# SkylerGao/MC_NeRF

Hardware: AMD Instinct MI355X
Metric: train rays/sec (coarse+fine, 64+128 samples) (higher is better)
Workload: dtype f16x3h; 1 GPU; Ball_Lego-shaped 110-view 800x800, coarse 4x128 @64 + fine 8x256 @128-grid, GLOBAL_OPTIM stage, fwd+bwd+allreduce+RAdam; precision=f16x3h, parallelism=dp1

## Files before the change

### mc_nerf_amd/csrc/mcnerf_x3.h

```cpp
#pragma once
#include "mcnerf_16.h"

#define MCNX3_SW 256.0f
#define MCNX3_SX 8.0f
#define MCNX3_SLABF 8
#define MCNX3_PF 2

#define MCNX3_WIDE_MIN 128
static inline constexpr int mcnx3_waves(int width) { return width >= MCNX3_WIDE_MIN ? 4 : 8; }

static inline int mcnx3_pad(int frags) { return (frags + MCNX3_SLABF - 1) / MCNX3_SLABF * MCNX3_SLABF; }
static inline Mcn16Stream mcnx3_repad(Mcn16Stream st) {
    int total = 0;
    for (int s = 0; s < st.nseg; ++s) {
        st.seg[s].first_frag = total;
        total += mcnx3_pad(st.seg[s].tiles * (st.seg[s].a.ksteps + st.seg[s].b.ksteps));
    }
    st.total_frags = total;
    return st;
}
static inline Mcn16Stream mcnx3_fwd_stream(const McnLayout& L) { return mcnx3_repad(mcn16_fwd_stream(L)); }
static inline Mcn16Stream mcnx3_bwd_stream(const McnLayout& L) { return mcnx3_repad(mcn16_bwd_stream(L)); }

static inline size_t mcnx3_slot_bytes(long long capacity, int width) { return 2 * mcn16_slot_bytes(capacity, width); }
static inline size_t mcnx3_enc_bytes(long long capacity) { return 2 * mcn16_enc_bytes(capacity); }
static inline size_t mcnx3_sh_bytes(long long capacity) { return (size_t)mcn16_cap_tiles(capacity) * 4096; }
static inline size_t mcnx3_dsh_bytes(long long capacity) { return 2 * mcn16_dsh_bytes(capacity); }

hipError_t mcnx3_launch_fwd(const Mcn16FwdArgs& a, hipStream_t st);
hipError_t mcnx3_launch_bwd(const Mcn16BwdArgs& a, hipStream_t st);
hipError_t mcnx3_launch_dw(const Mcn16DwArgs& a, hipStream_t st);
hipError_t mcnx3_launch_pack(const McnLayout& L, const float* params, void* packed_fwd, void* packed_bwd, unsigned* range_flags, hipStream_t st);

#ifdef __HIPCC__
typedef float f32x2_t __attribute__((ext_vector_type(2)));

__device__ __forceinline__ void mcnx3_split2(float a, float b, unsigned& hi, unsigned& lo) {
    const f16x2_t h = __builtin_convertvector((f32x2_t){a, b}, f16x2_t);
    const f32x2_t back = __builtin_convertvector(h, f32x2_t);
    const f16x2_t l = __builtin_convertvector((f32x2_t){a - back[0], b - back[1]}, f16x2_t);
    hi = __builtin_bit_cast(unsigned, h);
    lo = __builtin_bit_cast(unsigned, l);
}
__device__ __forceinline__ float mcnx3_val(unsigned hi, unsigned lo, int e) {
    const f16x2_t h = __builtin_bit_cast(f16x2_t, hi), l = __builtin_bit_cast(f16x2_t, lo);
    return (float)h[e] + (float)l[e];
}
template <int HI>
__device__ __forceinline__ float mcnx3_residual(float v, unsigned hw) {
    float r;
    if (HI) asm("v_fma_mix_f32 %0, %1, -1.0, %2 op_sel:[1,0,0] op_sel_hi:[1,0,0]" : "=v"(r) : "v"(hw), "v"(v));
    else asm("v_fma_mix_f32 %0, %1, -1.0, %2 op_sel_hi:[1,0,0]" : "=v"(r) : "v"(hw), "v"(v));
    return r;
}
__device__ __forceinline__ float mcnx3_relu(float x) {
    const int i = __builtin_bit_cast(int, x);
    return __builtin_bit_cast(float, i > 0 ? i : 0);
}
__device__ __forceinline__ f32x16 mcnx3_mfma(const u32x4_t& a, const u32x4_t& b, const f32x16& c) {
    return __builtin_amdgcn_mfma_f32_32x32x16_f16(__builtin_bit_cast(f16x8_t, a), __builtin_bit_cast(f16x8_t, b), c, 0, 0, 0);
}
__device__ __forceinline__ void mcnx3_mfma3(f32x16& acc, const u32x4_t& ah, const u32x4_t& al, const u32x4_t& bh, const u32x4_t& bl) {
    acc = mcnx3_mfma(al, bh, acc);
    acc = mcnx3_mfma(ah, bl, acc);
    acc = mcnx3_mfma(ah, bh, acc);
}

__device__ __forceinline__ void mcnx3_dma16(const char* ubase, unsigned voff, unsigned lds_dst) {
    unsigned keep;
    asm volatile("s_mov_b32 %0, m0\n\ts_mov_b32 m0, %3\n\ts_nop 0\n\tglobal_load_lds_dwordx4 %1, %2\n\ts_mov_b32 m0, %0"
                 : "=&s"(keep) : "v"(voff), "s"(ubase), "s"(lds_dst) : "memory");
}
template <int PPW>
__device__ __forceinline__ void mcnx3_ring_issue(Mcn16Ring& r) {
    const char* s = r.ubase + (size_t)r.src_slab * (MCN16_SLAB * 1024);
    const unsigned d = r.lds_base + r.issue_slot * (MCN16_SLAB * 1024) + r.lds_piece;
#pragma unroll
    for (int i = 0; i < PPW; ++i) mcnx3_dma16(s + i * 1024, r.voff, d + i * 1024);
    r.src_slab = (r.src_slab + 1 == r.n_slabs) ? 0 : r.src_slab + 1;
    r.issue_slot = (r.issue_slot + 1) & (MCN16_RING - 1);
}
template <int PPW>
__device__ __forceinline__ void mcnx3_ring_sync(Mcn16Ring& r) {
    asm volatile("s_waitcnt vmcnt(%0)\n\ts_barrier" ::"n"(PPW * (MCN16_AHEAD - 1)) : "memory");
    r.next_off = r.sync_slot * (MCN16_SLAB * 1024);
    r.sync_slot = (r.sync_slot + 1) & (MCN16_RING - 1);
    mcnx3_ring_issue<PPW>(r);
}
template <int PPW>
__device__ __forceinline__ void mcnx3_ring_start(Mcn16Ring& r, char* ring_lds, const void* packed, int n_slabs, int wave, int lane) {
    r.ubase = reinterpret_cast<const char*>(packed) + (PPW * wave) * 1024;
    r.voff = lane * 16;
    r.src = nullptr;
    r.lds_piece = (PPW * wave) * 1024;
    r.lds_base = (unsigned)reinterpret_cast<size_t>((mcn16_lds_ptr_t)ring_lds);
    r.src_slab = 0; r.n_slabs = n_slabs; r.issue_slot = 0; r.sync_slot = 0; r.next_off = 0;
#pragma unroll
    for (int i = 0; i < MCN16_AHEAD; ++i) mcnx3_ring_issue<PPW>(r);
    mcnx3_ring_sync<PPW>(r);
}
template <int F>
__host__ __device__ constexpr int mcnx3_sync_at(int q) {
    return (MCNX3_SLABF * q + MCNX3_SLABF - MCNX3_PF) < (F - 1) ? (MCNX3_SLABF * q + MCNX3_SLABF - MCNX3_PF) : (F - 1);
}
template <int F, int PPW>
__device__ __forceinline__ void mcnx3_before_mfma(Mcn16Ring& r, Mcn16Cursor& c, int f) {
    if ((f & (MCNX3_SLABF - 1)) == 0) c.cur = r.next_off;
    if (f == mcnx3_sync_at<F>(f / MCNX3_SLABF)) mcnx3_ring_sync<PPW>(r);
}
#define MCNX3_DMA_STEP 2
template <int PPW>
__device__ __forceinline__ void mcnx3_ring_piece(Mcn16Ring& r, int i) {
    switch (i) {
        case 0: asm volatile("global_load_lds_dwordx4 %0, %1" ::"v"(r.voff), "s"(r.piece_base) : "memory"); break;
        case 1: asm volatile("global_load_lds_dwordx4 %0, %1 offset:1024" ::"v"(r.voff), "s"(r.piece_base) : "memory"); break;
        case 2: asm volatile("global_load_lds_dwordx4 %0, %1 offset:2048" ::"v"(r.voff), "s"(r.piece_base) : "memory"); break;
        default: asm volatile("global_load_lds_dwordx4 %0, %1 offset:3072" ::"v"(r.voff), "s"(r.piece_base) : "memory"); break;
    }
// ... 53 lines not shown
```

### mc_nerf_amd/csrc/mlp_x3_bwd.hip

```cpp
#include "mcnerf_x3.h"
#include "mcnerf_launch.h"

#define MCNX3_BWD_PREF_MINW 256
#include <cstdlib>

template <int W>
struct BwdX3Smem {
    static constexpr int WAVES = mcnx3_waves(W);
    static constexpr int oW2 = MCN16_RING * MCN16_SLAB * 1024;
    static constexpr int oBarf = oW2 + W * 4;
    static constexpr int MW = W >= 64 ? W / 64 : 1;
    static constexpr int oMask = oBarf + 16 * 4;
    static constexpr int oIdx = oMask + WAVES * 3 * MW * 256;
    static constexpr int oIn = oIdx + WAVES * 256;
    static constexpr int total = oIn + (W >= 256 ? WAVES * 16 * 256 : 0);
};

template <int W, int KSTEPS, int NTILES, int MODE, int PPW, bool HI>
__device__ __forceinline__ void mcnx3_bwd_seg(Mcn16Ring& ring, char* smem, int lane,
                                              const u32x4_t (&inh)[W / 16], const u32x4_t (&inl)[W / 16],
                                              u32x4_t (&outh)[W / 16], u32x4_t (&outl)[W / 16],
                                              const unsigned (&mk)[W >= 64 ? W / 64 : 1], f32x16 (&acc2)[2], char* save_lane) {
    constexpr int KS = W / 16, F = NTILES * KSTEPS, G = 3 * KSTEPS;
    constexpr bool EPI = MODE != 3;
    constexpr int NIT = EPI ? (MODE == 0 ? 16 : 20) : 0;
    constexpr int START = (G >= NIT + 8) ? 3 : 0;
    constexpr int IPG = EPI ? (NIT + (G - START) - 1) / (G - START) : 1;
    constexpr int LASTA = EPI ? START + 14 / IPG : 0;
    constexpr int SBASE = START + 16, SSTR = (G - SBASE) / 4 > 0 ? (G - SBASE) / 4 : 1;
    constexpr bool STAG = (MODE == 1 || MODE == 2) && IPG == 1 && (G - SBASE) / 4 >= 2;
    constexpr int NITG = STAG ? 16 : NIT;
    constexpr int INIT_G = (G - 8) > LASTA ? (G - 8) : LASTA;
    constexpr int INIT_N = (INIT_G + 3 <= G - 1) ? 4 : 1;
    Mcn16Cursor cur;
    u32x4_t afh[MCNX3_PF], afl[MCNX3_PF];
    f32x16 acc[2];
    float v0 = 0.f, v1 = 0.f;
    unsigned wkeep = 0u;
    auto acc_init = [&](f32x16& a, int t, int q) {
        if (MODE == 2) {
            const f16x8_t h8 = __builtin_bit_cast(f16x8_t, outh[2 * t + (q >> 1)]), l8 = __builtin_bit_cast(f16x8_t, outl[2 * t + (q >> 1)]);
#pragma unroll
            for (int e = 0; e < 4; ++e) a[4 * q + e] = ((float)h8[4 * (q & 1) + e] + (float)l8[4 * (q & 1) + e]) * MCNX3_SW;
        } else {
#pragma unroll
            for (int e = 0; e < 4; ++e) a[4 * q + e] = 0.f;
        }
    };
    auto item = [&](const f32x16& a, int t, int i) {
        if (i < 16) {
            const int p = i >> 1;
            const unsigned bits = MODE != 0 ? ((mk[t >> 1] >> (8 * (t & 1) + 7 - p)) & 0x00010001u) : 0u;
            if ((i & 1) == 0) {
                v0 = a[2 * p] * (1.0f / MCNX3_SW);
                v1 = a[2 * p + 1] * (1.0f / MCNX3_SW);
                const unsigned w = Mcn16T<false>::pack(v0, v1);
                wkeep = w;
                outh[2 * t + (p >> 2)][p & 3] = MODE != 0 ? mcn16_pkmul(w, bits) : w;
            } else {
                const unsigned w = Mcn16T<false>::pack(mcnx3_residual<0>(v0, wkeep), mcnx3_residual<1>(v1, wkeep));
                outl[2 * t + (p >> 2)][p & 3] = MODE != 0 ? mcn16_pkmul(w, bits) : w;
            }
        } else {
            const int k = i - 16, s = 2 * t + (k & 1);
            if (k < 2) mcn16_ws_store(outh[s], reinterpret_cast<u32x4_t*>(save_lane + s * 1024));
            else if (!HI) mcn16_ws_store(outl[s], reinterpret_cast<u32x4_t*>(save_lane + (KS + s) * 1024));
        }
    };
    cur.cur = ring.next_off;
#pragma unroll
    for (int i = 0; i < MCNX3_PF; ++i)
        if (i < F) {
            afh[i] = *reinterpret_cast<const u32x4_t*>(smem + ring.next_off + i * 2048 + lane * 16);
            afl[i] = *reinterpret_cast<const u32x4_t*>(smem + ring.next_off + i * 2048 + 1024 + lane * 16);
        }
    if (EPI) {
#pragma unroll
        for (int q = 0; q < 4; ++q) acc_init(acc[0], 0, q);
    }
#pragma unroll
    for (int t = 0; t < NTILES; ++t) {
#pragma unroll
        for (int s = 0; s < KSTEPS; ++s) {
            const int f = t * KSTEPS + s;
            mcnx3_before_mfma_spread<F, PPW>(ring, cur, f);
            const u32x4_t a_h = afh[f % MCNX3_PF], a_l = afl[f % MCNX3_PF];
            if (f + MCNX3_PF < F) {
                const unsigned o = mcnx3_frag_off(ring, cur, f, f + MCNX3_PF) + lane * 16;
                afh[f % MCNX3_PF] = *reinterpret_cast<const u32x4_t*>(smem + o);
                afl[f % MCNX3_PF] = *reinterpret_cast<const u32x4_t*>(smem + o + 1024);
            }
#pragma unroll
            for (int g = 0; g < 3; ++g) {
                const int gap = 3 * s + g;
                if (EPI && t > 0 && gap >= START) {
#pragma unroll
                    for (int i = (gap - START) * IPG; i < (gap - START + 1) * IPG; ++i)
                        if (i < NITG) item(acc[(t - 1) & 1], t - 1, i);
                    if (STAG && gap >= SBASE && (gap - SBASE) / SSTR < 4 && (gap - SBASE) % SSTR == 0)
                        item(acc[(t - 1) & 1], t - 1, 16 + (gap - SBASE) / SSTR);
                }
                if (EPI && t + 1 < NTILES && gap >= INIT_G && gap < INIT_G + INIT_N) {
#pragma unroll
                    for (int q = 0; q < 4; ++q)
                        if (INIT_N == 1 || q == gap - INIT_G) acc_init(acc[(t + 1) & 1], t + 1, q);
                }
                mcnx3_gap_dma<F, PPW>(ring, 3 * f + g);
                __builtin_amdgcn_sched_barrier(0);
                if (EPI) acc[t & 1] = mcnx3_mfma(g == 0 ? a_l : a_h, g == 1 ? inl[s] : inh[s], acc[t & 1]);
                else acc2[t & 1] = mcnx3_mfma(g == 0 ? a_l : a_h, g == 1 ? inl[s] : inh[s], acc2[t & 1]);
                __builtin_amdgcn_sched_barrier(0);
            }
        }
    }
    mcnx3_layer_end<F, PPW>(ring);
    if (EPI) {
#pragma unroll
        for (int i = 0; i < NIT; ++i) item(acc[(NTILES - 1) & 1], NTILES - 1, i);
    }
}

template <int W, bool HI>
__global__ __launch_bounds__(64 * mcnx3_waves(W), mcnx3_waves(W) / 4) void mlp_x3_bwd_kernel(Mcn16BwdArgs a) {
    using SM = BwdX3Smem<W>;
    constexpr int PL = HI ? 1 : 2;
    constexpr int WAVES = mcnx3_waves(W), ROWS = 32 * WAVES, PPW = 16 / WAVES;
    constexpr int NT = W / 32, KS = W / 16, MW = W >= 64 ? W / 64 : 1;
    extern __shared__ __attribute__((aligned(16))) char smem[];
    const int tid = threadIdx.x, lane = tid & 63, wave = __builtin_amdgcn_readfirstlane(tid >> 6);
    const int m = lane & 31, h = lane >> 5;
    const int D = a.lay.depth, skip = a.lay.skip;
    const long long total = a.count ? (long long)min(*a.count, a.max_rows) : (long long)a.n_rays * a.S;
    if ((long long)blockIdx.x * ROWS >= total) return;

    float* sw2 = reinterpret_cast<float*>(smem + SM::oW2);
    for (int i = tid; i < W; i += 64 * WAVES) sw2[i] = a.params[a.lay.pWs2 + i];
    float* sbarf = reinterpret_cast<float*>(smem + SM::oBarf);
    if (tid < MCN_NFREQ) sbarf[tid] = a.barf_w[tid];
    const float gmax = __uint_as_float(*a.gmax_bits);
    const float sg = mcn16_grad_scale(gmax);
    const float inv_sg = 1.0f / sg;
    __syncthreads();

    struct In { int ray; float zg, jit; f32x4 o, go; float dx, dy, dz, ox, oy, oz; };
    auto gather = [&](int ray, int j) -> In {
        In r;
        r.ray = ray;
        r.zg = a.zgrid[ray * a.z_stride + j];
        r.jit = a.jitter ? a.jitter[ray] : 0.f;
        const size_t addr = (size_t)ray * a.S + j;
        r.o = *reinterpret_cast<const f32x4*>(a.out + addr * 4);
        r.go = *reinterpret_cast<const f32x4*>(a.d_out + addr * 4);
        r.dx = a.rays_d[ray * 3]; r.dy = a.rays_d[ray * 3 + 1]; r.dz = a.rays_d[ray * 3 + 2];
        r.ox = a.rays_o[ray * 3]; r.oy = a.rays_o[ray * 3 + 1]; r.oz = a.rays_o[ray * 3 + 2];
        return r;
    };
    auto row_of = [&](long long pass_) -> long long {
        const long long g_ = (pass_ * WAVES + wave) * 32 + m;
        return g_ < total ? g_ : total - 1;
    };
    constexpr bool PREFB = W >= MCNX3_BWD_PREF_MINW;
    constexpr int SLABS_FULL = (W / 32) * (W / 16) / MCNX3_SLABF;
    constexpr int SLABS_ENC = (2 * (W / 16) + MCNX3_SLABF - 1) / MCNX3_SLABF;
    constexpr int N_IDX = PPW * (2 * SLABS_FULL - 1) < 63 ? PPW * (2 * SLABS_FULL - 1) : 63;
    constexpr int N_TOP = PPW * (SLABS_FULL + SLABS_ENC - 1) < 63 ? PPW * (SLABS_FULL + SLABS_ENC - 1) : 63;
    const unsigned in_lds = (unsigned)reinterpret_cast<size_t>((mcn16_lds_ptr_t)smem) + SM::oIn + wave * (16 * 256);
    const float* in_rd = reinterpret_cast<const float*>(smem + SM::oIn + wave * (16 * 256)) + lane;
    auto gather_dma = [&](int ray, int j) {
        mcn16_dma4(a.zgrid + ray * a.z_stride + j, in_lds);
        if (a.jitter) mcn16_dma4(a.jitter + ray, in_lds + 256);
        const size_t addr = ((size_t)ray * a.S + j) * 4;
#pragma unroll
        for (int c = 0; c < 4; ++c) {
            mcn16_dma4(a.out + addr + c, in_lds + (2 + c) * 256);
            mcn16_dma4(a.d_out + addr + c, in_lds + (6 + c) * 256);
        }
#pragma unroll
        for (int c = 0; c < 3; ++c) {
            mcn16_dma4(a.rays_d + ray * 3 + c, in_lds + (10 + c) * 256);
            mcn16_dma4(a.rays_o + ray * 3 + c, in_lds + (13 + c) * 256);
// ... 95 lines not shown
                unsigned wh, wl;
                mcnx3_split2(v[0], v[1], wh, wl);
                dshh[s][d] = wh; dshl[s][d] = wl;
            }
        {
            char* e = reinterpret_cast<char*>(a.dsh_ws) + (size_t)tile * (PL * 2) * 1024 + lane * 16;
            mcn16_ws_store(dshh[0], reinterpret_cast<u32x4_t*>(e));
            mcn16_ws_store(dshh[1], reinterpret_cast<u32x4_t*>(e + 1024));
            if (!HI) {
                mcn16_ws_store(dshl[0], reinterpret_cast<u32x4_t*>(e + 2048));
                mcn16_ws_store(dshl[1], reinterpret_cast<u32x4_t*>(e + 3072));
            }
        }

        if (MASK_DMA) mask_read(mask_lane, mk_s, 0, D);
        else {
#pragma unroll
            for (int i = 0; i < MW; ++i) { mk_s[i] = mk0_s[i]; mk_c[i] = mk0_c[i]; mk_t[i] = mk0_t[i]; }
        }
        const long long pass_n = pass + gridDim.x;
        if (a.idx) {
            const long long gn = (pass_n * WAVES + wave) * 32 + (lane >> 1);
            mcn16_dma4(reinterpret_cast<const int*>(a.idx) + 2 * (gn < total ? gn : total - 1) + (lane & 1), idx_lds);
        }
        const bool want_rays = a.d_rays_o || a.d_rays_d;
        f32x4 shs[4];
#pragma unroll
        for (int q = 0; q < 4; ++q) shs[q] = f32x4{0.f, 0.f, 0.f, 0.f};
        if (PREFB && want_rays) {
#pragma unroll
            for (int q = 0; q < 4; ++q)
                shs[q] = *reinterpret_cast<const f32x4*>(reinterpret_cast<const char*>(a.sh_ws) + (size_t)tile * 4096 + q * 1024 + lane * 16);
        }
        u32x4_t xah[KS], xal[KS], xbh[KS], xbl[KS];
        f32x16 denc[2];
#pragma unroll
        for (int t = 0; t < 2; ++t)
#pragma unroll
            for (int e = 0; e < 16; ++e) denc[t][e] = 0.f;
#pragma unroll
        for (int s = 0; s < KS; ++s) {
            const f32x4 wa = *reinterpret_cast<const f32x4*>(w2_h + 16 * s), wb = *reinterpret_cast<const f32x4*>(w2_h + 16 * s + 8);
            const int t = s >> 1;
#pragma unroll
            for (int d = 0; d < 4; ++d) {
                const float va = (d < 2 ? wa[2 * d] : wb[2 * d - 4]) * dsg, vb = (d < 2 ? wa[2 * d + 1] : wb[2 * d - 3]) * dsg;
                const int i = 4 * (s & 1) + d;
                const unsigned bits = (mk_s[t >> 1] >> (8 * (t & 1) + 7 - i)) & 0x00010001u;
                unsigned wh, wl;
                mcnx3_split2(va, vb, wh, wl);
                xah[s][d] = mcn16_pkmul(wh, bits);
                xal[s][d] = mcn16_pkmul(wl, bits);
            }
            mcn16_ws_store(xah[s], reinterpret_cast<u32x4_t*>(dy_lane + (size_t)D * a.slot_bytes + s * 1024));
            if (!HI) mcn16_ws_store(xal[s], reinterpret_cast<u32x4_t*>(dy_lane + (size_t)D * a.slot_bytes + (KS + s) * 1024));
        }
        if (D >= 2) mask_issue(mask_lane, D - 2, buf_of(D - 2));
        unsigned mpend[MW];
        if (!MASK_DMA && D >= 2) mask_read(mask_lane, mpend, 0, D - 2);
        mcnx3_bwd_seg<W, KS, NT, 0, PPW, HI>(ring, smem, lane, xah, xal, xbh, xbl, mk_s, denc, nullptr);
        if (MASK_DMA) mask_read(mask_lane, mk_c, 1, D + 1);
        {
            u32x4_t dih[KS], dil[KS];
            dih[0] = dshh[0]; dih[1] = dshh[1]; dil[0] = dshl[0]; dil[1] = dshl[1];
            mcnx3_bwd_seg<W, 2, NT, 1, PPW, HI>(ring, smem, lane, dih, dil, xah, xal, mk_c, denc, dy_lane + (size_t)(D + 1) * a.slot_bytes);
        }
        if (D >= 3) mask_issue(mask_lane, D - 3, buf_of(D - 3));
        if (MASK_DMA) mask_read(mask_lane, mk_t, 2, D - 1);
        mcnx3_bwd_seg<W, KS, NT, 2, PPW, HI>(ring, smem, lane, xah, xal, xbh, xbl, mk_t, denc, dy_lane + (size_t)(D - 1) * a.slot_bytes);
        auto trunk_masks = [&](int l) {
            if (MASK_DMA) {
                if (l >= 3) mask_issue(mask_lane, l - 3, buf_of(l - 3));
                mask_read(mask_lane, mk_t, buf_of(l - 1), l - 1);
            } else {
#pragma unroll
                for (int i = 0; i < MW; ++i) mk_t[i] = mpend[i];
                if (l >= 2) mask_read(mask_lane, mpend, 0, l - 2);
            }
            if (l == 1 && pass_n * ROWS < total) {
                const unsigned* mln = mask_lane_of(pass_n);
                mask_issue(mln, D, 0); mask_issue(mln, D + 1, 1); mask_issue(mln, D - 1, 2);
                if (!MASK_DMA) { mask_read(mln, mk0_s, 0, D); mask_read(mln, mk0_c, 1, D + 1); mask_read(mln, mk0_t, 2, D - 1); }
            }
        };
        auto next_rows = [&]() {
            asm volatile("s_waitcnt vmcnt(%0)" ::"n"(N_IDX) : "memory");
            int rn, jn;
            if (a.idx) {
                const int2 rj = *reinterpret_cast<const int2*>(smem + SM::oIdx + wave * 256 + m * 8);
                rn = rj.x; jn = rj.y;
            } else {
                const long long gn = row_of(pass_n);
                rn = (int)(gn / a.S); jn = (int)(gn - (long long)rn * a.S);
            }
            gather_dma(rn, jn);
            ray_n = rn;
        };
        for (int l = D - 1; l >= 1; l -= 2) {
            if (PREFB && l == 1) next_rows();
            trunk_masks(l);
            if (l == skip) mcnx3_bwd_seg<W, KS, 2, 3, PPW, HI>(ring, smem, lane, xbh, xbl, xah, xal, mk_t, denc, nullptr);
            mcnx3_bwd_seg<W, KS, NT, 1, PPW, HI>(ring, smem, lane, xbh, xbl, xah, xal, mk_t, denc, dy_lane + (size_t)(l - 1) * a.slot_bytes);
            if (l - 1 >= 1) {
                if (PREFB && l - 1 == 1) next_rows();
                trunk_masks(l - 1);
                if (l - 1 == skip) mcnx3_bwd_seg<W, KS, 2, 3, PPW, HI>(ring, smem, lane, xah, xal, xbh, xbl, mk_t, denc, nullptr);
                mcnx3_bwd_seg<W, KS, NT, 1, PPW, HI>(ring, smem, lane, xah, xal, xbh, xbl, mk_t, denc, dy_lane + (size_t)(l - 2) * a.slot_bytes);
            } else {
#pragma unroll
                for (int s = 0; s < KS; ++s) { xbh[s] = xah[s]; xbl[s] = xal[s]; }
            }
        }
        In nxt = cur;
        if (PREFB && D < 2) {
            next_rows();
        }
        if (!PREFB) {
            int rn, jn;
            if (a.idx) {
                const int2 rj = *reinterpret_cast<const int2*>(smem + SM::oIdx + wave * 256 + m * 8);
                rn = rj.x; jn = rj.y;
            } else {
                const long long gn = row_of(pass_n);
                rn = (int)(gn / a.S); jn = (int)(gn - (long long)rn * a.S);
            }
            nxt = gather(rn, jn);
        }
        if (!PREFB && want_rays) {
#pragma unroll
            for (int q = 0; q < 4; ++q)
                shs[q] = *reinterpret_cast<const f32x4*>(reinterpret_cast<const char*>(a.sh_ws) + (size_t)tile * 4096 + q * 1024 + lane * 16);
        }
        mcnx3_bwd_seg<W, KS, 2, 3, PPW, HI>(ring, smem, lane, xbh, xbl, xah, xal, mk_t, denc, nullptr);
        auto settle = [&]() {
            if (PREFB && D >= 2) return;
            asm volatile("s_waitcnt vmcnt(0)" ::: "memory");
            asm volatile("" : "+v"(nxt.ray), "+v"(nxt.zg), "+v"(nxt.jit), "+v"(nxt.o), "+v"(nxt.go));
            asm volatile("" : "+v"(nxt.dx), "+v"(nxt.dy), "+v"(nxt.dz), "+v"(nxt.ox), "+v"(nxt.oy), "+v"(nxt.oz));
            if (!MASK_DMA) {
#pragma unroll
                for (int i = 0; i < MW; ++i) asm volatile("" : "+v"(mk0_s[i]), "+v"(mk0_c[i]), "+v"(mk0_t[i]));
            }
        };

        if (want_rays) {
            auto dch = [&](int ch) -> float {
                const int hh = (ch >> 2) & 1;
                const float v = denc[ch >> 5][4 * ((ch >> 3) & 3) + (ch & 3)];
                return (h == hh) ? v : 0.f;
            };
            float dpos[3];
#pragma unroll
            for (int ax = 0; ax < 3; ++ax) {
                float acc = dch(ax);
                float S[MCN_NFREQ], C[MCN_NFREQ];
                mcn_sincos_octaves<MCN_NFREQ>(p[ax], S, C);
#pragma unroll
                for (int f = 0; f < MCN_NFREQ; ++f) {
                    const float k = (float)(1 << f) * sbarf[f];
                    acc = fmaf(k * C[f], dch(3 + 20 * ax + f), acc);
                    acc = fmaf(-k * S[f], dch(3 + 20 * ax + 10 + f), acc);
                }
                dpos[ax] = acc * (1.0f / MCNX3_SW);
            }
            float ddir[3] = {0.f, 0.f, 0.f};
            {
                const float C1 = 0.4886025119029199f, C20 = 1.0925484305920792f, C22 = 0.31539156525252005f, C24 = 0.5462742152960396f;
                const float gx[9] = {0.f, 0.f, 0.f, -C1, C20 * y, 0.f, -2.f * C22 * x, -C20 * z, 2.f * C24 * x};
                const float gy[9] = {0.f, -C1, 0.f, 0.f, C20 * x, -C20 * z, -2.f * C22 * y, 0.f, -2.f * C24 * y};
                const float gz[9] = {0.f, 0.f, C1, 0.f, 0.f, -C20 * y, 4.f * C22 * z, -C20 * x, 0.f};
#pragma unroll
                for (int r = 0; r < 16; ++r) {
                    const float v = shs[r >> 2][r & 3];
                    const int n0 = 8 * (r >> 2) + (r & 3), n1 = n0 + 4;
                    const float kx = h ? (n1 < MCN_NSH ? dpre[n1 / 9] * gx[n1 % 9] : 0.f) : (n0 < MCN_NSH ? dpre[n0 / 9] * gx[n0 % 9] : 0.f);
                    const float ky = h ? (n1 < MCN_NSH ? dpre[n1 / 9] * gy[n1 % 9] : 0.f) : (n0 < MCN_NSH ? dpre[n0 / 9] * gy[n0 % 9] : 0.f);
                    const float kz = h ? (n1 < MCN_NSH ? dpre[n1 / 9] * gz[n1 % 9] : 0.f) : (n0 < MCN_NSH ? dpre[n0 / 9] * gz[n0 % 9] : 0.f);
                    ddir[0] = fmaf(kx, v, ddir[0]); ddir[1] = fmaf(ky, v, ddir[1]); ddir[2] = fmaf(kz, v, ddir[2]);
                }
            }
            float red[6];
#pragma unroll
            for (int c = 0; c < 3; ++c) {
                const float dp = dpos[c] + __shfl_xor(dpos[c], 32);
                const float dd = ddir[c] + __shfl_xor(ddir[c], 32);
                red[c] = dp * inv_sg;
// ... 40 lines not shown
```

### mc_nerf_amd/csrc/mlp_x3_fwd.hip

```cpp
#include "mcnerf_x3.h"
#include "mcnerf_launch.h"

template <int W>
struct FwdX3Smem {
    static constexpr int oBias = MCN16_RING * MCN16_SLAB * 1024;
    static constexpr int oW2 = oBias + (MCN_MAXD + 2) * W * 4;
    static constexpr int oBc2 = oW2 + W * 4;
    static constexpr int oIdx = oBc2 + 32 * 4;
    static constexpr int oIn = oIdx + mcnx3_waves(W) * 256;
    static constexpr int total = oIn + mcnx3_waves(W) * 8 * 256;
};

template <int W, int SV, int KENC, int KHID, int EPI, int PPW>
__device__ __forceinline__ void mcnx3_layer(Mcn16Ring& ring, char* smem, int lane,
                                            const u32x4_t (&ench)[MCN16_ENCKS], const u32x4_t (&encl)[MCN16_ENCKS],
                                            const u32x4_t (&inh)[W / 16], const u32x4_t (&inl)[W / 16],
                                            u32x4_t (&outh)[W / 16], u32x4_t (&outl)[W / 16], const float* bias_h,
                                            const float* w2_h, float& dot, char* save_lane, unsigned* mask_lane) {
    constexpr bool SAVE = SV != 0, HI = SV == 2;
    constexpr int NT = W / 32, KS = W / 16, KTOT = KENC + KHID, F = NT * KTOT, MW = W >= 64 ? W / 64 : 1;
    constexpr int G = 3 * KTOT;
    constexpr bool HAS2 = SAVE || EPI == 1;
    constexpr int IPW = HAS2 ? 3 : 2;
    constexpr int NST = SAVE ? (HI ? 2 : 4) : 0;
    constexpr int NIT = 8 * IPW + NST;
    constexpr int NWI = 8 * IPW;
    constexpr int ROOM = G - 3 - 2 * NST;
    constexpr int IPGA = ROOM > 0 ? (NWI + ROOM - 1) / ROOM : 99;
    constexpr bool STAG = SAVE && IPGA <= 2;
    constexpr int START = STAG ? 3 : (G >= NIT + 4 ? 3 : 0);
    constexpr int IPG = STAG ? IPGA : (NIT + (G - START) - 1) / (G - START);
    constexpr int NITG = STAG ? NWI : NIT;
    constexpr int LASTG = START + (NITG + IPG - 1) / IPG - 1;
    constexpr int SBASE = LASTG + 1, SSTR = STAG ? (G - SBASE) / NST : 1;
    constexpr int BIAS_G = (G - 6) > LASTG ? (G - 6) : LASTG;
    Mcn16Cursor cur;
    unsigned mw[MW];
#pragma unroll
    for (int i = 0; i < MW; ++i) mw[i] = 0u;
    u32x4_t afh[MCNX3_PF], afl[MCNX3_PF];
    f32x16 acc[2];
    unsigned mb = 0u;
    float v0 = 0.f, v1 = 0.f;
    unsigned wkeep = 0u;
    auto bias_init = [&](f32x16& a, int t) {
#pragma unroll
        for (int q = 0; q < 4; ++q) {
            const f32x4 b = *reinterpret_cast<const f32x4*>(bias_h + 32 * t + 8 * q);
#pragma unroll
            for (int e = 0; e < 4; ++e) a[4 * q + e] = b[e];
        }
    };
    auto item = [&](const f32x16& a, int t, int i) {
        if (i < 8 * IPW) {
            const int p = i / IPW, ph = i % IPW;
            if (ph == 0) {
                v0 = mcnx3_relu(a[2 * p] * (1.0f / MCNX3_SW));
                v1 = mcnx3_relu(a[2 * p + 1] * (1.0f / MCNX3_SW));
                const unsigned w = Mcn16T<false>::pack(v0, v1);
                wkeep = w;
                outh[2 * t + (p >> 2)][p & 3] = w;
            } else if (ph == IPW - 1) {
                outl[2 * t + (p >> 2)][p & 3] = Mcn16T<false>::pack(mcnx3_residual<0>(v0, wkeep), mcnx3_residual<1>(v1, wkeep));
            } else {
                if (SAVE) {
                    mb = (p == 0) ? mcn16_nz(wkeep) : ((mb << 1) | mcn16_nz(wkeep));
                    if (p == 7) mw[t >> 1] |= mb << (8 * (t & 1));
                }
                if (EPI == 1) {
                    const f32x2_t ww = *reinterpret_cast<const f32x2_t*>(w2_h + 32 * t + 8 * (p >> 1) + 2 * (p & 1));
                    dot = fmaf(v0, ww[0], dot);
                    dot = fmaf(v1, ww[1], dot);
                }
            }
        } else if (SAVE) {
            const int k = i - 8 * IPW;
            const int s = 2 * t + (k & 1);
            if (k < 2) mcn16_ws_store(outh[s], reinterpret_cast<u32x4_t*>(save_lane + s * 1024));
            else mcn16_ws_store(outl[s], reinterpret_cast<u32x4_t*>(save_lane + (KS + s) * 1024));
        }
    };
    cur.cur = ring.next_off;
#pragma unroll
    for (int i = 0; i < MCNX3_PF; ++i)
        if (i < F) {
            afh[i] = *reinterpret_cast<const u32x4_t*>(smem + ring.next_off + i * 2048 + lane * 16);
            afl[i] = *reinterpret_cast<const u32x4_t*>(smem + ring.next_off + i * 2048 + 1024 + lane * 16);
        }
    bias_init(acc[0], 0);
#pragma unroll
    for (int t = 0; t < NT; ++t) {
#pragma unroll
        for (int s = 0; s < KTOT; ++s) {
            const int f = t * KTOT + s;
            mcnx3_before_mfma_spread<F, PPW>(ring, cur, f);
            const u32x4_t a_h = afh[f % MCNX3_PF], a_l = afl[f % MCNX3_PF];
            if (f + MCNX3_PF < F) {
                const unsigned o = mcnx3_frag_off(ring, cur, f, f + MCNX3_PF) + lane * 16;
                afh[f % MCNX3_PF] = *reinterpret_cast<const u32x4_t*>(smem + o);
                afl[f % MCNX3_PF] = *reinterpret_cast<const u32x4_t*>(smem + o + 1024);
            }
            const u32x4_t b_h = s < KENC ? ench[s < KENC ? s : 0] : inh[s >= KENC ? s - KENC : 0];
            const u32x4_t b_l = s < KENC ? encl[s < KENC ? s : 0] : inl[s >= KENC ? s - KENC : 0];
#pragma unroll
            for (int g = 0; g < 3; ++g) {
                const int gap = 3 * s + g;
                if (t > 0 && gap >= START) {
#pragma unroll
                    for (int i = (gap - START) * IPG; i < (gap - START + 1) * IPG; ++i)
                        if (i < NITG) item(acc[(t - 1) & 1], t - 1, i);
                    if (STAG && gap >= SBASE && (gap - SBASE) / SSTR < NST && (gap - SBASE) % SSTR == 0)
                        item(acc[(t - 1) & 1], t - 1, 8 * IPW + (gap - SBASE) / SSTR);
                }
                if (gap == BIAS_G && t + 1 < NT) bias_init(acc[(t + 1) & 1], t + 1);
                mcnx3_gap_dma<F, PPW>(ring, 3 * f + g);
                __builtin_amdgcn_sched_barrier(0);
                acc[t & 1] = mcnx3_mfma(g == 0 ? a_l : a_h, g == 1 ? b_l : b_h, acc[t & 1]);
                __builtin_amdgcn_sched_barrier(0);
            }
        }
    }
    mcnx3_layer_end<F, PPW>(ring);
#pragma unroll
    for (int i = 0; i < NIT; ++i) item(acc[(NT - 1) & 1], NT - 1, i);
    if (SAVE) {
#pragma unroll
        for (int i = 0; i < MW; ++i) mcn16_ws_store(mw[i], mask_lane + i);
    }
}


template <int W, int SV>
__global__ __launch_bounds__(64 * mcnx3_waves(W), mcnx3_waves(W) / 4) void mlp_x3_fwd_kernel(Mcn16FwdArgs a) {
    using SM = FwdX3Smem<W>;
    constexpr bool SAVE = SV != 0, HI = SV == 2;
    constexpr int PL = HI ? 1 : 2;
    constexpr int WAVES = mcnx3_waves(W), ROWS = 32 * WAVES, PPW = 16 / WAVES;
    constexpr int KS = W / 16, MW = W >= 64 ? W / 64 : 1;
    constexpr float SXW = MCNX3_SX * MCNX3_SW;
    extern __shared__ __attribute__((aligned(16))) char smem[];
    const int tid = threadIdx.x, lane = tid & 63, wave = __builtin_amdgcn_readfirstlane(tid >> 6);
    const int m = lane & 31, h = lane >> 5;
    const int D = a.lay.depth, skip = a.lay.skip;
    const long long total = a.count ? (long long)min(*a.count, a.max_rows) : (long long)a.n_rays * a.S;
    if ((long long)blockIdx.x * ROWS >= total) return;

    float* sbias = reinterpret_cast<float*>(smem + SM::oBias);
    float* sw2 = reinterpret_cast<float*>(smem + SM::oW2);
    float* sbc2 = reinterpret_cast<float*>(smem + SM::oBc2);
    for (int l = 0; l < D; ++l)
        for (int i = tid; i < W; i += 64 * WAVES) sbias[l * W + i] = a.params[a.lay.pB[l] + i] * SXW;
    for (int i = tid; i < W; i += 64 * WAVES) {
        sbias[D * W + i] = a.params[a.lay.pBs1 + i] * SXW;
        sbias[(D + 1) * W + i] = a.params[a.lay.pBc1 + i] * SXW;
        sw2[i] = a.params[a.lay.pWs2 + i];
    }
    if (tid < 32) {
        const int row = tid < MCN_NSH ? mcn_sh_row(tid, a.lay.sh_deg) : -1;
        sbc2[tid] = row >= 0 ? a.params[a.lay.pBc2 + row] * SXW : 0.f;
    }
    const float bs2 = a.params[a.lay.pBs2];
    float bw[MCN_NFREQ];
#pragma unroll
    for (int f = 0; f < MCN_NFREQ; ++f) bw[f] = a.barf_w[f];
    __syncthreads();

    constexpr bool PREF = WAVES == 4;
    constexpr int SLABS_FULL = (W / 32) * (W / 16) / MCNX3_SLABF, SLABS_L0 = ((W / 32) * MCN16_ENCKS + MCNX3_SLABF - 1) / MCNX3_SLABF;
    constexpr int SLABS_SH2 = (W / 16 + MCNX3_SLABF - 1) / MCNX3_SLABF;
    constexpr int N_IDX = PPW * (SLABS_L0 + SLABS_FULL - 1) < 63 ? PPW * (SLABS_L0 + SLABS_FULL - 1) : 63;
    constexpr int N_TOP = PPW * (SLABS_FULL + SLABS_SH2 - 1) < 63 ? PPW * (SLABS_FULL + SLABS_SH2 - 1) : 63;
    const unsigned idx_lds = (unsigned)reinterpret_cast<size_t>((mcn16_lds_ptr_t)smem) + SM::oIdx + wave * 256;
    const unsigned in_lds = (unsigned)reinterpret_cast<size_t>((mcn16_lds_ptr_t)smem) + SM::oIn + wave * (8 * 256);
    const float* in_rd = reinterpret_cast<const float*>(smem + SM::oIn + wave * (8 * 256)) + lane;
    auto row_of = [&](long long pass_) -> long long {
        const long long g_ = (pass_ * WAVES + wave) * 32 + m;
        return g_ < total ? g_ : total - 1;
    };
    auto gather_dma = [&](int ray_, int j_) {
        mcn16_dma4(a.zgrid + ray_ * a.z_stride + j_, in_lds);
        if (a.jitter) mcn16_dma4(a.jitter + ray_, in_lds + 256);
#pragma unroll
        for (int c = 0; c < 3; ++c) {
            mcn16_dma4(a.rays_d + ray_ * 3 + c, in_lds + (2 + c) * 256);
            mcn16_dma4(a.rays_o + ray_ * 3 + c, in_lds + (5 + c) * 256);
        }
    };
    int ray_n = 0, j_n = 0;
    {
        const long long gc0 = row_of(blockIdx.x);
        if (a.idx) { const int2 rj = a.idx[gc0]; ray_n = rj.x; j_n = rj.y; }
// ... 19 lines not shown
        int ray, j;
        float zv, dx, dy, dz, ox, oy, oz;
        if (PREF) {
            ray = ray_n; j = j_n;
            asm volatile("s_waitcnt vmcnt(%0)" ::"n"(N_TOP) : "memory");
            zv = in_rd[0];
            if (a.jitter) zv = __fadd_rn(zv, in_rd[64]);
            dx = in_rd[2 * 64]; dy = in_rd[3 * 64]; dz = in_rd[4 * 64];
            ox = in_rd[5 * 64]; oy = in_rd[6 * 64]; oz = in_rd[7 * 64];
        } else {
            if (a.idx) { const int2 rj = a.idx[gc]; ray = rj.x; j = rj.y; }
            else { ray = (int)(gc / a.S); j = (int)(gc - (long long)ray * a.S); }
            zv = a.zgrid[ray * a.z_stride + j];
            if (a.jitter) zv = __fadd_rn(zv, a.jitter[ray]);
            dx = a.rays_d[ray * 3 + 0]; dy = a.rays_d[ray * 3 + 1]; dz = a.rays_d[ray * 3 + 2];
            ox = a.rays_o[ray * 3 + 0]; oy = a.rays_o[ray * 3 + 1]; oz = a.rays_o[ray * 3 + 2];
        }
        float p[3];
        p[0] = __fadd_rn(ox, __fmul_rn(dx, zv));
        p[1] = __fadd_rn(oy, __fmul_rn(dy, zv));
        p[2] = __fadd_rn(oz, __fmul_rn(dz, zv));
        if (PREF && a.idx) {
            const long long gn = (pass_n * WAVES + wave) * 32 + (lane >> 1);
            mcn16_dma4(reinterpret_cast<const int*>(a.idx) + 2 * (gn < total ? gn : total - 1) + (lane & 1), idx_lds);
        }
        const int addr = ray * a.S + j;
        u32x4_t ench[MCN16_ENCKS], encl[MCN16_ENCKS];
        {
            float E[64];
            mcnx3_encode_values(p, bw, E);
#pragma unroll
            for (int s = 0; s < MCN16_ENCKS; ++s)
#pragma unroll
                for (int d = 0; d < 4; ++d) {
                    const int c0 = mcn16_chan(s, 0, 2 * d), c1 = mcn16_chan(s, 0, 2 * d + 1);
                    unsigned wh, wl;
                    mcnx3_split2((h ? E[c0 + 4] : E[c0]) * MCNX3_SX, (h ? E[c1 + 4] : E[c1]) * MCNX3_SX, wh, wl);
                    ench[s][d] = wh; encl[s][d] = wl;
                }
        }
        char* act_lane = SAVE ? reinterpret_cast<char*>(a.act_ws) + (size_t)tile * (PL * KS) * 1024 + lane * 16 : nullptr;
        unsigned* mask_lane = SAVE ? a.mask_ws + ((size_t)tile * 64 + lane) * MW : nullptr;
        if (SAVE) {
            char* e = reinterpret_cast<char*>(a.enc_ws) + (size_t)tile * (PL * MCN16_ENCKS) * 1024 + lane * 16;
#pragma unroll
            for (int s = 0; s < MCN16_ENCKS; ++s) {
                mcn16_ws_store(ench[s], reinterpret_cast<u32x4_t*>(e + s * 1024));
                if (!HI) mcn16_ws_store(encl[s], reinterpret_cast<u32x4_t*>(e + (MCN16_ENCKS + s) * 1024));
            }
        }

        u32x4_t xah[KS], xal[KS], xbh[KS], xbl[KS];
        float dot = 0.f;
        mcnx3_layer<W, SV, MCN16_ENCKS, 0, 0, PPW>(ring, smem, lane, ench, encl, xah, xal, xbh, xbl, bias_h, nullptr, dot, act_lane, mask_lane);
        for (int l = 1; l < D; l += 2) {
            char* sl = SAVE ? act_lane + (size_t)l * a.slot_bytes : nullptr;
            unsigned* ml = SAVE ? mask_lane + (size_t)l * a.mask_slot_words : nullptr;
            if (l == skip) mcnx3_layer<W, SV, MCN16_ENCKS, KS, 0, PPW>(ring, smem, lane, ench, encl, xbh, xbl, xah, xal, bias_h + l * W, nullptr, dot, sl, ml);
            else mcnx3_layer<W, SV, 0, KS, 0, PPW>(ring, smem, lane, ench, encl, xbh, xbl, xah, xal, bias_h + l * W, nullptr, dot, sl, ml);
            if (l + 1 < D) {
                sl = SAVE ? act_lane + (size_t)(l + 1) * a.slot_bytes : nullptr;
                ml = SAVE ? mask_lane + (size_t)(l + 1) * a.mask_slot_words : nullptr;
                if (l + 1 == skip) mcnx3_layer<W, SV, MCN16_ENCKS, KS, 0, PPW>(ring, smem, lane, ench, encl, xah, xal, xbh, xbl, bias_h + (l + 1) * W, nullptr, dot, sl, ml);
                else mcnx3_layer<W, SV, 0, KS, 0, PPW>(ring, smem, lane, ench, encl, xah, xal, xbh, xbl, bias_h + (l + 1) * W, nullptr, dot, sl, ml);
            } else {
#pragma unroll
                for (int s = 0; s < KS; ++s) { xbh[s] = xah[s]; xbl[s] = xal[s]; }
            }
        }
        mcnx3_layer<W, SV, 0, KS, 1, PPW>(ring, smem, lane, ench, encl, xbh, xbl, xah, xal, bias_h + D * W, w2_h, dot,
                                            SAVE ? act_lane + (size_t)D * a.slot_bytes : nullptr, SAVE ? mask_lane + (size_t)D * a.mask_slot_words : nullptr);
        if (PREF) {
            asm volatile("s_waitcnt vmcnt(%0)" ::"n"(N_IDX) : "memory");
            if (a.idx) {
                const int2 rj = *reinterpret_cast<const int2*>(smem + SM::oIdx + wave * 256 + m * 8);
                ray_n = rj.x; j_n = rj.y;
            } else {
                const long long gn = row_of(pass_n);
                ray_n = (int)(gn / a.S); j_n = (int)(gn - (long long)ray_n * a.S);
            }
            gather_dma(ray_n, j_n);
        }
        mcnx3_layer<W, SV, 0, KS, 0, PPW>(ring, smem, lane, ench, encl, xbh, xbl, xah, xal, bias_h + (D + 1) * W, nullptr, dot,
                                            SAVE ? act_lane + (size_t)(D + 1) * a.slot_bytes : nullptr, SAVE ? mask_lane + (size_t)(D + 1) * a.mask_slot_words : nullptr);
        f32x16 acc;
#pragma unroll
        for (int q = 0; q < 4; ++q) {
            const f32x4 b = *reinterpret_cast<const f32x4*>(sbc2 + 8 * q + 4 * h);
#pragma unroll
            for (int e = 0; e < 4; ++e) acc[4 * q + e] = b[e];
        }
        {
            Mcn16Cursor cur;
#pragma unroll
            for (int s = 0; s < KS; ++s) {
                mcnx3_before_mfma<KS, PPW>(ring, cur, s);
                const unsigned o = cur.cur + (s & (MCNX3_SLABF - 1)) * 2048 + lane * 16;
                const u32x4_t a_h = *reinterpret_cast<const u32x4_t*>(smem + o);
                const u32x4_t a_l = *reinterpret_cast<const u32x4_t*>(smem + o + 1024);
                mcnx3_mfma3(acc, a_h, a_l, xah[s], xal[s]);
            }
        }
#pragma unroll
        for (int e = 0; e < 16; ++e) acc[e] *= 1.0f / SXW;
        if (SAVE) {
            char* e = reinterpret_cast<char*>(a.sh_ws) + (size_t)tile * 4096 + lane * 16;
#pragma unroll
            for (int q = 0; q < 4; ++q)
                mcn16_ws_store(f32x4{acc[4 * q], acc[4 * q + 1], acc[4 * q + 2], acc[4 * q + 3]}, reinterpret_cast<f32x4*>(e + q * 1024));
        }
        float bas[9];
        mcn_sh_basis(dx, dy, dz, bas);
        float pre[3] = {0.f, 0.f, 0.f};
#pragma unroll
        for (int r = 0; r < 16; ++r) {
            const int n0 = 8 * (r >> 2) + (r & 3), n1 = n0 + 4;
            const float b0 = n0 < MCN_NSH ? bas[n0 % 9] : 0.f, b1 = n1 < MCN_NSH ? bas[n1 % 9] : 0.f;
            const float contrib = acc[r] * (h ? b1 : b0);
            const int c0 = n0 / 9, c1 = n1 / 9;
#pragma unroll
            for (int c = 0; c < 3; ++c) {
                const bool in0 = n0 < MCN_NSH && c0 == c, in1 = n1 < MCN_NSH && c1 == c;
                if (in0 && in1) pre[c] += contrib;
                else if (in0) pre[c] += h ? 0.f : contrib;
                else if (in1) pre[c] += h ? contrib : 0.f;
            }
        }
        const float sigma = (dot + __shfl_xor(dot, 32)) * (1.0f / MCNX3_SX) + bs2;
        f32x4 o;
        o[0] = sigma;
#pragma unroll
        for (int c = 0; c < 3; ++c) {
            const float pc = pre[c] + __shfl_xor(pre[c], 32);
            o[1 + c] = 1.0f / (1.0f + expf(-pc));
        }
        if (valid && h == 0) *reinterpret_cast<f32x4*>(a.out + (size_t)addr * 4) = o;
// ... 12 lines not shown
```

Before: 1.091 million rays/s.

## Pin ping-pong activation buffers to AGPR/VGPR homes in wide MLP layers

New measurement: 1.097 million rays/s (median of 6 runs). No clear change (+0.6%).

```diff
diff --git a/mc_nerf_amd/csrc/mcnerf_x3.h b/mc_nerf_amd/csrc/mcnerf_x3.h
--- a/mc_nerf_amd/csrc/mcnerf_x3.h
+++ b/mc_nerf_amd/csrc/mcnerf_x3.h
@@ -64,6 +64,12 @@
     acc = mcnx3_mfma(al, bh, acc);
     acc = mcnx3_mfma(ah, bl, acc);
     acc = mcnx3_mfma(ah, bh, acc);
+}
+
+template <int HOME>
+__device__ __forceinline__ void mcnx3_home_pin(u32x4_t& v) {
+    if (HOME == 2) asm volatile("" : "+a"(v));
+    else if (HOME == 1) asm volatile("" : "+v"(v));
 }
 
 __device__ __forceinline__ void mcnx3_dma16(const char* ubase, unsigned voff, unsigned lds_dst) {
diff --git a/mc_nerf_amd/csrc/mlp_x3_bwd.hip b/mc_nerf_amd/csrc/mlp_x3_bwd.hip
--- a/mc_nerf_amd/csrc/mlp_x3_bwd.hip
+++ b/mc_nerf_amd/csrc/mlp_x3_bwd.hip
@@ -16,7 +16,7 @@
     static constexpr int total = oIn + (W >= 256 ? WAVES * 16 * 256 : 0);
 };
 
-template <int W, int KSTEPS, int NTILES, int MODE, int PPW, bool HI>
+template <int W, int KSTEPS, int NTILES, int MODE, int PPW, bool HI, int HOME>
 __device__ __forceinline__ void mcnx3_bwd_seg(Mcn16Ring& ring, char* smem, int lane,
                                               const u32x4_t (&inh)[W / 16], const u32x4_t (&inl)[W / 16],
                                               u32x4_t (&outh)[W / 16], u32x4_t (&outl)[W / 16],
@@ -57,9 +57,11 @@
                 const unsigned w = Mcn16T<false>::pack(v0, v1);
                 wkeep = w;
                 outh[2 * t + (p >> 2)][p & 3] = MODE != 0 ? mcn16_pkmul(w, bits) : w;
+                if (HOME == 2 && (p & 3) == 3) mcnx3_home_pin<2>(outh[2 * t + (p >> 2)]);
             } else {
                 const unsigned w = Mcn16T<false>::pack(mcnx3_residual<0>(v0, wkeep), mcnx3_residual<1>(v1, wkeep));
                 outl[2 * t + (p >> 2)][p & 3] = MODE != 0 ? mcn16_pkmul(w, bits) : w;
+                if (HOME == 2 && (p & 3) == 3) mcnx3_home_pin<2>(outl[2 * t + (p >> 2)]);
             }
         } else {
             const int k = i - 16, s = 2 * t + (k & 1);
@@ -117,6 +119,8 @@
     if (EPI) {
 #pragma unroll
         for (int i = 0; i < NIT; ++i) item(acc[(NTILES - 1) & 1], NTILES - 1, i);
+#pragma unroll
+        for (int s = 0; s < KS; ++s) { mcnx3_home_pin<HOME>(outh[s]); mcnx3_home_pin<HOME>(outl[s]); }
     }
 }
 
@@ -126,6 +130,8 @@
     constexpr int PL = HI ? 1 : 2;
     constexpr int WAVES = mcnx3_waves(W), ROWS = 32 * WAVES, PPW = 16 / WAVES;
     constexpr int NT = W / 32, KS = W / 16, MW = W >= 64 ? W / 64 : 1;
+    constexpr bool HOMES = W >= 256;
+    constexpr int HA = HOMES ? 2 : 0, HB = HOMES ? 1 : 0;
     extern __shared__ __attribute__((aligned(16))) char smem[];
     const int tid = threadIdx.x, lane = tid & 63, wave = __builtin_amdgcn_readfirstlane(tid >> 6);
     const int m = lane & 31, h = lane >> 5;
@@ -327,22 +333,23 @@
                 xah[s][d] = mcn16_pkmul(wh, bits);
                 xal[s][d] = mcn16_pkmul(wl, bits);
             }
+            mcnx3_home_pin<HA>(xah[s]); mcnx3_home_pin<HA>(xal[s]);
             mcn16_ws_store(xah[s], reinterpret_cast<u32x4_t*>(dy_lane + (size_t)D * a.slot_bytes + s * 1024));
             if (!HI) mcn16_ws_store(xal[s], reinterpret_cast<u32x4_t*>(dy_lane + (size_t)D * a.slot_bytes + (KS + s) * 1024));
         }
         if (D >= 2) mask_issue(mask_lane, D - 2, buf_of(D - 2));
         unsigned mpend[MW];
         if (!MASK_DMA && D >= 2) mask_read(mask_lane, mpend, 0, D - 2);
-        mcnx3_bwd_seg<W, KS, NT, 0, PPW, HI>(ring, smem, lane, xah, xal, xbh, xbl, mk_s, denc, nullptr);
+        mcnx3_bwd_seg<W, KS, NT, 0, PPW, HI, HB>(ring, smem, lane, xah, xal, xbh, xbl, mk_s, denc, nullptr);
         if (MASK_DMA) mask_read(mask_lane, mk_c, 1, D + 1);
         {
             u32x4_t dih[KS], dil[KS];
             dih[0] = dshh[0]; dih[1] = dshh[1]; dil[0] = dshl[0]; dil[1] = dshl[1];
-            mcnx3_bwd_seg<W, 2, NT, 1, PPW, HI>(ring, smem, lane, dih, dil, xah, xal, mk_c, denc, dy_lane + (size_t)(D + 1) * a.slot_bytes);
+            mcnx3_bwd_seg<W, 2, NT, 1, PPW, HI, HA>(ring, smem, lane, dih, dil, xah, xal, mk_c, denc, dy_lane + (size_t)(D + 1) * a.slot_bytes);
         }
         if (D >= 3) mask_issue(mask_lane, D - 3, buf_of(D - 3));
         if (MASK_DMA) mask_read(mask_lane, mk_t, 2, D - 1);
-        mcnx3_bwd_seg<W, KS, NT, 2, PPW, HI>(ring, smem, lane, xah, xal, xbh, xbl, mk_t, denc, dy_lane + (size_t)(D - 1) * a.slot_bytes);
+        mcnx3_bwd_seg<W, KS, NT, 2, PPW, HI, HB>(ring, smem, lane, xah, xal, xbh, xbl, mk_t, denc, dy_lane + (size_t)(D - 1) * a.slot_bytes);
         auto trunk_masks = [&](int l) {
             if (MASK_DMA) {
                 if (l >= 3) mask_issue(mask_lane, l - 3, buf_of(l - 3));
@@ -374,14 +381,14 @@
         for (int l = D - 1; l >= 1; l -= 2) {
             if (PREFB && l == 1) next_rows();
             trunk_masks(l);
-            if (l == skip) mcnx3_bwd_seg<W, KS, 2, 3, PPW, HI>(ring, smem, lane, xbh, xbl, xah, xal, mk_t, denc, nullptr);
-            mcnx3_bwd_seg<W, KS, NT, 1, PPW, HI>(ring, smem, lane, xbh, xbl, xah, xal, mk_t, denc, dy_lane + (size_t)(l - 1) * a.slot_bytes);
+            if (l == skip) mcnx3_bwd_seg<W, KS, 2, 3, PPW, HI, 0>(ring, smem, lane, xbh, xbl, xah, xal, mk_t, denc, nullptr);
+            mcnx3_bwd_seg<W, KS, NT, 1, PPW, HI, HA>(ring, smem, lane, xbh, xbl, xah, xal, mk_t, denc, dy_lane + (size_t)(l - 1) * a.slot_bytes);
             if (l - 1 >= 1) {
                 if (PREFB && l - 1 == 1) next_rows();
                 trunk_masks(l - 1);
-                if (l - 1 == skip) mcnx3_bwd_seg<W, KS, 2, 3, PPW, HI>(ring, smem, lane, xah, xal, xbh, xbl, mk_t, denc, nullptr);
-                mcnx3_bwd_seg<W, KS, NT, 1, PPW, HI>(ring, smem, lane, xah, xal, xbh, xbl, mk_t, denc, dy_lane + (size_t)(l - 2) * a.slot_bytes);
-            } else {
+                if (l - 1 == skip) mcnx3_bwd_seg<W, KS, 2, 3, PPW, HI, 0>(ring, smem, lane, xah, xal, xbh, xbl, mk_t, denc, nullptr);
+                mcnx3_bwd_seg<W, KS, NT, 1, PPW, HI, HB>(ring, smem, lane, xah, xal, xbh, xbl, mk_t, denc, dy_lane + (size_t)(l - 2) * a.slot_bytes);
+            } else if (!HOMES) {
 #pragma unroll
                 for (int s = 0; s < KS; ++s) { xbh[s] = xah[s]; xbl[s] = xal[s]; }
             }
@@ -406,7 +413,8 @@
             for (int q = 0; q < 4; ++q)
                 shs[q] = *reinterpret_cast<const f32x4*>(reinterpret_cast<const char*>(a.sh_ws) + (size_t)tile * 4096 + q * 1024 + lane * 16);
         }
-        mcnx3_bwd_seg<W, KS, 2, 3, PPW, HI>(ring, smem, lane, xbh, xbl, xah, xal, mk_t, denc, nullptr);
+        if (HOMES && D >= 2 && !(D & 1)) mcnx3_bwd_seg<W, KS, 2, 3, PPW, HI, 0>(ring, smem, lane, xah, xal, xbh, xbl, mk_t, denc, nullptr);
+        else mcnx3_bwd_seg<W, KS, 2, 3, PPW, HI, 0>(ring, smem, lane, xbh, xbl, xah, xal, mk_t, denc, nullptr);
         auto settle = [&]() {
             if (PREFB && D >= 2) return;
             asm volatile("s_waitcnt vmcnt(0)" ::: "memory");
diff --git a/mc_nerf_amd/csrc/mlp_x3_fwd.hip b/mc_nerf_amd/csrc/mlp_x3_fwd.hip
--- a/mc_nerf_amd/csrc/mlp_x3_fwd.hip
+++ b/mc_nerf_amd/csrc/mlp_x3_fwd.hip
@@ -11,7 +11,7 @@
     static constexpr int total = oIn + mcnx3_waves(W) * 8 * 256;
 };
 
-template <int W, int SV, int KENC, int KHID, int EPI, int PPW>
+template <int W, int SV, int KENC, int KHID, int EPI, int PPW, int HOME>
 __device__ __forceinline__ void mcnx3_layer(Mcn16Ring& ring, char* smem, int lane,
                                             const u32x4_t (&ench)[MCN16_ENCKS], const u32x4_t (&encl)[MCN16_ENCKS],
                                             const u32x4_t (&inh)[W / 16], const u32x4_t (&inl)[W / 16],
@@ -60,8 +60,10 @@
                 const unsigned w = Mcn16T<false>::pack(v0, v1);
                 wkeep = w;
                 outh[2 * t + (p >> 2)][p & 3] = w;
+                if (HOME == 2 && (p & 3) == 3) mcnx3_home_pin<2>(outh[2 * t + (p >> 2)]);
             } else if (ph == IPW - 1) {
                 outl[2 * t + (p >> 2)][p & 3] = Mcn16T<false>::pack(mcnx3_residual<0>(v0, wkeep), mcnx3_residual<1>(v1, wkeep));
+                if (HOME == 2 && (p & 3) == 3) mcnx3_home_pin<2>(outl[2 * t + (p >> 2)]);
             } else {
                 if (SAVE) {
                     mb = (p == 0) ? mcn16_nz(wkeep) : ((mb << 1) | mcn16_nz(wkeep));
@@ -71,6 +73,7 @@
                     const f32x2_t ww = *reinterpret_cast<const f32x2_t*>(w2_h + 32 * t + 8 * (p >> 1) + 2 * (p & 1));
                     dot = fmaf(v0, ww[0], dot);
                     dot = fmaf(v1, ww[1], dot);
+                    if (HOME != 0) asm volatile("" : "+v"(dot));
                 }
             }
         } else if (SAVE) {
@@ -127,6 +130,8 @@
 #pragma unroll
         for (int i = 0; i < MW; ++i) mcn16_ws_store(mw[i], mask_lane + i);
     }
+#pragma unroll
+    for (int s = 0; s < KS; ++s) { mcnx3_home_pin<HOME>(outh[s]); mcnx3_home_pin<HOME>(outl[s]); }
 }
 
 
@@ -137,6 +142,8 @@
     constexpr int PL = HI ? 1 : 2;
     constexpr int WAVES = mcnx3_waves(W), ROWS = 32 * WAVES, PPW = 16 / WAVES;
     constexpr int KS = W / 16, MW = W >= 64 ? W / 64 : 1;
+    constexpr bool HOMES = W >= 256;
+    constexpr int HA = HOMES ? 1 : 0, HB = HOMES ? 2 : 0;
     constexpr float SXW = MCNX3_SX * MCNX3_SW;
     extern __shared__ __attribute__((aligned(16))) char smem[];
     const int tid = threadIdx.x, lane = tid & 63, wave = __builtin_amdgcn_readfirstlane(tid >> 6);
@@ -262,23 +269,44 @@
 
         u32x4_t xah[KS], xal[KS], xbh[KS], xbl[KS];
         float dot = 0.f;
-        mcnx3_layer<W, SV, MCN16_ENCKS, 0, 0, PPW>(ring, smem, lane, ench, encl, xah, xal, xbh, xbl, bias_h, nullptr, dot, act_lane, mask_lane);
-        for (int l = 1; l < D; l += 2) {
-            char* sl = SAVE ? act_lane + (size_t)l * a.slot_bytes : nullptr;
-            unsigned* ml = SAVE ? mask_lane + (size_t)l * a.mask_slot_words : nullptr;
-            if (l == skip) mcnx3_layer<W, SV, MCN16_ENCKS, KS, 0, PPW>(ring, smem, lane, ench, encl, xbh, xbl, xah, xal, bias_h + l * W, nullptr, dot, sl, ml);
-            else mcnx3_layer<W, SV, 0, KS, 0, PPW>(ring, smem, lane, ench, encl, xbh, xbl, xah, xal, bias_h + l * W, nullptr, dot, sl, ml);
-            if (l + 1 < D) {
+        if (HOMES) {
+            mcnx3_layer<W, SV, MCN16_ENCKS, 0, 0, PPW, HA>(ring, smem, lane, ench, encl, xbh, xbl, xah, xal, bias_h, nullptr, dot, act_lane, mask_lane);
+            for (int l = 1;; l += 2) {
+                char* sl = SAVE ? act_lane + (size_t)l * a.slot_bytes : nullptr;
+                unsigned* ml = SAVE ? mask_lane + (size_t)l * a.mask_slot_words : nullptr;
+                if (l >= D) {
+#pragma unroll
+                    for (int s = 0; s < KS; ++s) {
+                        xbh[s] = xah[s]; xbl[s] = xal[s];
+                        mcnx3_home_pin<HB>(xbh[s]); mcnx3_home_pin<HB>(xbl[s]);
+                    }
+                } else if (l == skip) mcnx3_layer<W, SV, MCN16_ENCKS, KS, 0, PPW, HB>(ring, smem, lane, ench, encl, xah, xal, xbh, xbl, bias_h + l * W, nullptr, dot, sl, ml);
+                else mcnx3_layer<W, SV, 0, KS, 0, PPW, HB>(ring, smem, lane, ench, encl, xah, xal, xbh, xbl, bias_h + l * W, nullptr, dot, sl, ml);
+                if (l + 1 >= D) break;
                 sl = SAVE ? act_lane + (size_t)(l + 1) * a.slot_bytes : nullptr;
                 ml = SAVE ? mask_lane + (size_t)(l + 1) * a.mask_slot_words : nullptr;
-                if (l + 1 == skip) mcnx3_layer<W, SV, MCN16_ENCKS, KS, 0, PPW>(ring, smem, lane, ench, encl, xah, xal, xbh, xbl, bias_h + (l + 1) * W, nullptr, dot, sl, ml);
-                else mcnx3_layer<W, SV, 0, KS, 0, PPW>(ring, smem, lane, ench, encl, xah, xal, xbh, xbl, bias_h + (l + 1) * W, nullptr, dot, sl, ml);
-            } else {
-#pragma unroll
-                for (int s = 0; s < KS; ++s) { xbh[s] = xah[s]; xbl[s] = xal[s]; }
-            }
-        }
-        mcnx3_layer<W, SV, 0, KS, 1, PPW>(ring, smem, lane, ench, encl, xbh, xbl, xah, xal, bias_h + D * W, w2_h, dot,
+                if (l + 1 == skip) mcnx3_layer<W, SV, MCN16_ENCKS, KS, 0, PPW, HA>(ring, smem, lane, ench, encl, xbh, xbl, xah, xal, bias_h + (l + 1) * W, nullptr, dot, sl, ml);
+                else mcnx3_layer<W, SV, 0, KS, 0, PPW, HA>(ring, smem, lane, ench, encl, xbh, xbl, xah, xal, bias_h + (l + 1) * W, nullptr, dot, sl, ml);
+            }
+        } else {
+            mcnx3_layer<W, SV, MCN16_ENCKS, 0, 0, PPW, 0>(ring, smem, lane, ench, encl, xah, xal, xbh, xbl, bias_h, nullptr, dot, act_lane, mask_lane);
+            for (int l = 1; l < D; l += 2) {
+                char* sl = SAVE ? act_lane + (size_t)l * a.slot_bytes : nullptr;
+                unsigned* ml = SAVE ? mask_lane + (size_t)l * a.mask_slot_words : nullptr;
+                if (l == skip) mcnx3_layer<W, SV, MCN16_ENCKS, KS, 0, PPW, 0>(ring, smem, lane, ench, encl, xbh, xbl, xah, xal, bias_h + l * W, nullptr, dot, sl, ml);
+                else mcnx3_layer<W, SV, 0, KS, 0, PPW, 0>(ring, smem, lane, ench, encl, xbh, xbl, xah, xal, bias_h + l * W, nullptr, dot, sl, ml);
+                if (l + 1 < D) {
+                    sl = SAVE ? act_lane + (size_t)(l + 1) * a.slot_bytes : nullptr;
+                    ml = SAVE ? mask_lane + (size_t)(l + 1) * a.mask_slot_words : nullptr;
+                    if (l + 1 == skip) mcnx3_layer<W, SV, MCN16_ENCKS, KS, 0, PPW, 0>(ring, smem, lane, ench, encl, xah, xal, xbh, xbl, bias_h + (l + 1) * W, nullptr, dot, sl, ml);
+                    else mcnx3_layer<W, SV, 0, KS, 0, PPW, 0>(ring, smem, lane, ench, encl, xah, xal, xbh, xbl, bias_h + (l + 1) * W, nullptr, dot, sl, ml);
+                } else {
+#pragma unroll
+                    for (int s = 0; s < KS; ++s) { xbh[s] = xah[s]; xbl[s] = xal[s]; }
+                }
+            }
+        }
+        mcnx3_layer<W, SV, 0, KS, 1, PPW, HA>(ring, smem, lane, ench, encl, xbh, xbl, xah, xal, bias_h + D * W, w2_h, dot,
                                             SAVE ? act_lane + (size_t)D * a.slot_bytes : nullptr, SAVE ? mask_lane + (size_t)D * a.mask_slot_words : nullptr);
         if (PREF) {
             asm volatile("s_waitcnt vmcnt(%0)" ::"n"(N_IDX) : "memory");
@@ -291,7 +319,7 @@
             }
             gather_dma(ray_n, j_n);
         }
-        mcnx3_layer<W, SV, 0, KS, 0, PPW>(ring, smem, lane, ench, encl, xbh, xbl, xah, xal, bias_h + (D + 1) * W, nullptr, dot,
+        mcnx3_layer<W, SV, 0, KS, 0, PPW, HA>(ring, smem, lane, ench, encl, xbh, xbl, xah, xal, bias_h + (D + 1) * W, nullptr, dot,
                                             SAVE ? act_lane + (size_t)(D + 1) * a.slot_bytes : nullptr, SAVE ? mask_lane + (size_t)(D + 1) * a.mask_slot_words : nullptr);
         f32x16 acc;
 #pragma unroll
```
